# RoyAPTX4869/RaLD

Hardware: AMD Instinct MI355X
Metric: denoising steps/sec (whole node) (higher is better)
Workload: dtype bf16

## Files before the change

include/rald_hip.h:

```cpp
#ifndef RALD_HIP_H
#define RALD_HIP_H
#include <stdint.h>
#ifdef __cplusplus
extern "C" {
#endif

const char* rald_last_error(void);
int rald_version(void);
int rald_build_flags(void);
int64_t rald_debug_f16_saturation_count(int32_t reset);
int rald_debug_poison_lds(void* stream);

typedef struct rald_dit rald_dit;

typedef struct rald_dit_config {
    int32_t n_latents;
    int32_t channels;
    int32_t depth;
    int32_t n_heads;
    int32_t d_head;
    int32_t t_channels;
    int32_t context_dim;
    int32_t n_cond_tokens;
    int32_t with_radar_enc;
// ... 170 lines not shown
typedef struct rald_lidar rald_lidar;
int rald_lidar_create(const rald_lidar_config* cfg, rald_lidar** out);
void rald_lidar_destroy(rald_lidar* h);
int64_t rald_lidar_workspace_bytes(const rald_lidar_config* cfg, int32_t batch, int64_t total_points);
int rald_lidar_crop(const rald_lidar* h, const float* points, int32_t in_stride, const int64_t* offsets, int32_t batch, float* out,
                    int32_t* counts, void* workspace, int64_t workspace_bytes, void* stream);
int rald_lidar_voxelize(const rald_lidar* h, const float* points, const int64_t* offsets, const int32_t* counts, int32_t batch,
                        int32_t to_polar, float* polar_out, float* voxels, int32_t* coords, int32_t* num_points, int32_t* kept_keys,
                        int32_t* voxel_counts, void* workspace, int64_t workspace_bytes, void* stream);
int rald_lidar_queries(const rald_lidar* h, const float* points, const int64_t* offsets, int32_t batch, int32_t num_samples,
                       int32_t in_num, const int64_t* sample_idx, const double* u_in, const int64_t* voxel_idx, const double* u_out,
                       const int64_t* empty_rank, const int32_t* coords, const int32_t* kept_keys, const int32_t* voxel_counts,
                       float* lidar_points, float* query_points, float* query_labels, void* workspace, int64_t workspace_bytes,
                       void* stream);

int rald_op_gemm_nt(const void* A, int64_t lda, int64_t strideA, const void* B, int64_t ldb, int64_t strideB,
                    void* C, int64_t ldc, int64_t strideC, const float* bias, int32_t M, int32_t N, int32_t K,
                    int32_t batch, float alpha, int32_t epilogue, void* stream);
int rald_op_gemm_nt2(const void* A, int64_t lda, int64_t strideA, int64_t strideA2, const void* B, int64_t ldb, int64_t strideB, int64_t strideB2,
                     void* C, int64_t ldc, int64_t strideC, int64_t strideC2, const float* bias, int32_t M, int32_t N, int32_t K, int32_t batch,
                     int32_t batch2, float alpha, int32_t epilogue, void* stream);
int rald_op_gemm_nt_256(const void* A, int64_t lda, const void* B, int64_t ldb, void* C, int64_t ldc, const float* bias, int32_t M, int32_t N,
                        int32_t K, float alpha, int32_t alpha_ncols, int32_t epilogue, int32_t persistent, int32_t max_workgroups, void* stream);
int rald_op_gemm_tn(const void* A_bf16, int64_t lda, const void* B_bf16, int64_t ldb, float* C, int64_t ldc, float* colsum, int32_t M, int32_t N1,
                    int32_t N2, void* workspace, int64_t workspace_bytes, void* stream);
int rald_op_conv3d_wgrad(const void* dy_bf16, const void* x_bf16, float* dW, float* dbias, int32_t B, int32_t ID, int32_t IH, int32_t IW, int32_t Cin,
                         int32_t Cout, int32_t stride, int32_t pad, void* workspace, int64_t workspace_bytes, void* stream);
int64_t rald_op_gemm_tn_workspace_bytes(int32_t M, int32_t N1, int32_t N2);
int64_t rald_op_conv3d_wgrad_workspace_bytes(int32_t B, int32_t ID, int32_t IH, int32_t IW, int32_t Cin, int32_t Cout, int32_t stride, int32_t pad);
int rald_op_patches27(const float* cube, int32_t cube_ch, void* out_bf16, int32_t B, int32_t D, int32_t H, int32_t W, void* stream);
int rald_op_transpose(const void* in, int32_t in_is_bf16, int64_t ld_in, int64_t stride_in, int64_t stride_in2, void* out_bf16, int64_t ld_out,
                      int64_t stride_out, int64_t stride_out2, int32_t rows, int32_t cols, int32_t batch, int32_t batch2, void* stream);
int rald_op_ln_mod_bwd(const float* x, const float* dh, const float* scale, int64_t gstride, int32_t rows_per_group, float add_one, float eps,
                       int64_t rows, int32_t D, float* dx_accum, void* dx_bf16_out, float* dscale_accum, float* dshift_accum, void* stream);
int rald_op_geglu_fwd(const void* u_bf16, void* hid_bf16, int64_t M, int32_t inner, void* stream);
int rald_op_geglu_bwd(const void* u_bf16, const void* dhid_bf16, void* du_bf16, int64_t M, int32_t inner, void* stream);
int rald_op_colsum(const void* X, int32_t is_bf16, int64_t ld, int64_t M, int32_t N, float* out_accum, void* stream);
int rald_op_row_lse(const float* S, int64_t rows, int32_t cols, float scale, float* lse, void* stream);
int rald_op_rowdot_heads(const void* dO_bf16, const void* O_bf16, int64_t M, int32_t heads, int32_t nq, float* delta, void* stream);
int rald_op_attn_bwd_elem(const float* S, const float* dP, const float* lse, const float* delta, int64_t batch, int32_t R, int32_t Ccols,
                          int64_t vbatch_stride, int32_t vstride, float scale, int32_t by_col, void* P_bf16, void* dS_bf16, void* stream);
int rald_op_sgemm_acc(const float* A, int64_t lda, int32_t trans_a, const float* B, int64_t ldb, int32_t trans_b, float* C, int64_t ldc, int32_t M,
                      int32_t N, int32_t K, float alpha, void* stream);
int rald_op_silu_fwd(const float* x, float* y, int64_t n, void* stream);
int rald_op_silu_bwd(const float* x_pre, const float* dy, float* dx, int64_t n, void* stream);
int rald_op_posemb(const float* t, float* out, int32_t n, int32_t channels, void* stream);
// ... 129 lines not shown
```

rald_amd/_handles.py:

```python
from __future__ import annotations

import ctypes as C
import os
from typing import Dict, Iterable, Optional, Sequence, Tuple

import torch

from . import _lib
from ._lib import DitConfig, check, lib


def _stream() -> int:
    return torch.cuda.current_stream().cuda_stream


def _opt(t: Optional[torch.Tensor]) -> Optional[int]:
    return t.data_ptr() if t is not None else None


def _need_cuda(t: torch.Tensor, what: str) -> None:
    if not t.is_cuda:
        raise RuntimeError(f"rald_amd: {what} must live on the GPU (cuda tensor); this package has no CPU path")


# ... 316 lines not shown
    sB = B.stride(0) if B.dim() == 3 else 0
    nc = N // 2 if epilogue == 3 else N
    if epilogue == 2:
        out = C_inout
    else:
        shape = (batch, M, nc) if batched else (M, nc)
        out = torch.empty(shape, device=A.device, dtype=torch.float16 if epilogue == 5 else (torch.bfloat16 if epilogue in (0, 3, 4) else torch.float32))
    sC = out.stride(0) if out.dim() == 3 else 0
    check(lib().rald_op_gemm_nt(A.data_ptr(), A.stride(-2), sA, B.data_ptr(), B.stride(-2), sB, out.data_ptr(), out.stride(-2), sC, _opt(bias), M, N,
                                K, batch, alpha, epilogue, _stream()))
    return out


def op_gemm_nt_256(A: torch.Tensor, B: torch.Tensor, out: torch.Tensor, bias: Optional[torch.Tensor] = None, epilogue: int = 0, alpha: float = 1.0,
                   alpha_ncols: int = 1 << 30, persistent: int = 1, max_workgroups: int = 1 << 30) -> torch.Tensor:
    (M, K), N = A.shape, B.shape[0]
    assert A.dtype == B.dtype == out.dtype == torch.bfloat16 and A.stride(1) == B.stride(1) == out.stride(1) == 1
    assert out.shape == (M, N // 2 if epilogue == 3 else N) and B.shape[1] == K
    check(lib().rald_op_gemm_nt_256(A.data_ptr(), A.stride(0), B.data_ptr(), B.stride(0), out.data_ptr(), out.stride(0), _opt(bias), M, N, K,
                                    alpha, int(alpha_ncols), int(epilogue), int(persistent), int(max_workgroups), _stream()))
    return out


def op_gemm_tn(A: torch.Tensor, B: torch.Tensor, C_inout: torch.Tensor, colsum: Optional[torch.Tensor] = None, atomics: bool = True) -> torch.Tensor:
    M, N1 = A.shape
    N2 = B.shape[1]
    assert A.dtype == torch.bfloat16 and B.dtype == torch.bfloat16 and C_inout.dtype == torch.float32 and B.shape[0] == M
    assert A.stride(1) == 1 and B.stride(1) == 1 and C_inout.stride(1) == 1 and C_inout.shape == (N1, N2)
    ws, nbytes = None, 0
    if not atomics:
        nbytes = lib().rald_op_gemm_tn_workspace_bytes(M, N1, N2)
        ws = _scratch(nbytes, A.device)
    check(lib().rald_op_gemm_tn(A.data_ptr(), A.stride(0), B.data_ptr(), B.stride(0), C_inout.data_ptr(), C_inout.stride(0),
                                _opt(colsum), M, N1, N2, _opt(ws), nbytes, _stream()))
    return C_inout


def op_gemm_resid_ln(A: torch.Tensor, W: torch.Tensor, bias: torch.Tensor, x: torch.Tensor, g: torch.Tensor, b: torch.Tensor,
                     gstride: int = 0, rows_per_group: int = 1 << 30, add_one: float = 0.0, eps: float = 1e-5) -> torch.Tensor:
    M, K = A.shape
    h = torch.empty(M, 512, device=A.device, dtype=torch.bfloat16)
    check(lib().rald_op_gemm_resid_ln(A.data_ptr(), A.stride(0), W.data_ptr(), W.stride(0), bias.data_ptr(),
                                      x.data_ptr(), h.data_ptr(), g.data_ptr(), b.data_ptr(), gstride,
                                      rows_per_group, add_one, eps, M, K, _stream()))
    return h

# ... 368 lines not shown
```

rald_amd/csrc/api.hip:

```cpp
#include <cstdlib>
#include <cstring>

#include "ae.h"
#include "dit.h"
#include "lidar.h"
#include "radar_dsp.h"
#include "radar_points.h"

using namespace rald;

struct rald_dit { Dit impl; };
struct rald_ae { Ae impl; };

extern "C" {

const char* rald_last_error(void) { return rald::last_error(); }
int rald_version(void) { return 3; }
int rald_build_flags(void) { return 0; }

int64_t rald_debug_f16_saturation_count(int32_t reset) {
    unsigned a = 0, b = 0;
    if (hipDeviceSynchronize() != hipSuccess) return -1;
    if (f16_saturation_gemm(&a, reset != 0) || f16_saturation_attn(&b, reset != 0)) return -1;
    return (int64_t)a + (int64_t)b;
// ... 482 lines not shown
                    void* C, int64_t ldc, int64_t strideC, const float* bias, int32_t M, int32_t N, int32_t K,
                    int32_t batch, float alpha, int32_t epilogue, void* stream) {
    RALD_CHECK(A && B && C, "rald_op_gemm_nt: null pointer");
    GemmArgs g;
    g.A = (const bf16*)A; g.lda = lda; g.strideA = strideA; g.B = (const bf16*)B; g.ldb = ldb; g.strideB = strideB;
    g.C = C; g.ldc = ldc; g.strideC = strideC; g.bias = bias; g.M = M; g.N = N; g.K = K; g.batch = batch; g.alpha = alpha; g.alpha_ncols = 1 << 30; g.flags = 0;
    return gemm_nt(g, epilogue, (hipStream_t)stream);
}
int rald_op_gemm_nt2(const void* A, int64_t lda, int64_t strideA, int64_t strideA2, const void* B, int64_t ldb, int64_t strideB, int64_t strideB2,
                     void* C, int64_t ldc, int64_t strideC, int64_t strideC2, const float* bias, int32_t M, int32_t N, int32_t K, int32_t batch,
                     int32_t batch2, float alpha, int32_t epilogue, void* stream) {
    RALD_CHECK(A && B && C, "rald_op_gemm_nt2: null pointer");
    GemmArgs g = gemm_args((const bf16*)A, lda, (const bf16*)B, ldb, C, ldc, bias, M, N, K);
    g.strideA = strideA; g.strideB = strideB; g.strideC = strideC; g.batch = batch; g.alpha = alpha;
    g.batch2 = batch2; g.strideA2 = strideA2; g.strideB2 = strideB2; g.strideC2 = strideC2;
    return gemm_nt(g, epilogue, (hipStream_t)stream);
}
int rald_op_gemm_nt_256(const void* A, int64_t lda, const void* B, int64_t ldb, void* C, int64_t ldc, const float* bias, int32_t M, int32_t N,
                        int32_t K, float alpha, int32_t alpha_ncols, int32_t epilogue, int32_t persistent, int32_t max_workgroups, void* stream) {
    RALD_CHECK(A && B && C, "rald_op_gemm_nt_256: null pointer");
    GemmArgs g = gemm_args((const bf16*)A, lda, (const bf16*)B, ldb, C, ldc, bias, M, N, K);
    g.alpha = alpha; g.alpha_ncols = alpha_ncols;
    return gemm_nt_256_test(g, epilogue, persistent, max_workgroups, (hipStream_t)stream);
}
int rald_op_gemm_tn(const void* A_bf16, int64_t lda, const void* B_bf16, int64_t ldb, float* C, int64_t ldc, float* colsum, int32_t M, int32_t N1,
                    int32_t N2, void* workspace, int64_t workspace_bytes, void* stream) {
    return gemm_tn((const bf16*)A_bf16, lda, (const bf16*)B_bf16, ldb, C, ldc, colsum, M, N1, N2, (hipStream_t)stream, (float*)workspace, workspace_bytes / 4);
}
int rald_op_conv3d_wgrad(const void* dy_bf16, const void* x_bf16, float* dW, float* dbias, int32_t B, int32_t ID, int32_t IH, int32_t IW, int32_t Cin,
                         int32_t Cout, int32_t stride, int32_t pad, void* workspace, int64_t workspace_bytes, void* stream) {
    return conv3d_wgrad_tn((const bf16*)dy_bf16, (const bf16*)x_bf16, dW, dbias, B, ID, IH, IW, Cin, Cout, stride, pad, (hipStream_t)stream, (float*)workspace,
                           workspace_bytes / 4);
}
int64_t rald_op_gemm_tn_workspace_bytes(int32_t M, int32_t N1, int32_t N2) { return 4 * gemm_tn_workspace_floats(M, N1, N2); }
int64_t rald_op_conv3d_wgrad_workspace_bytes(int32_t B, int32_t ID, int32_t IH, int32_t IW, int32_t Cin, int32_t Cout, int32_t stride, int32_t pad) {
    return 4 * conv3d_wgrad_workspace_floats(B, ID, IH, IW, Cin, Cout, stride, pad);
}
int rald_op_patches27(const float* cube, int32_t cube_ch, void* out_bf16, int32_t B, int32_t D, int32_t H, int32_t W, void* stream) {
    return patches27(cube, cube_ch, (bf16*)out_bf16, B, D, H, W, (hipStream_t)stream);
}
int rald_op_transpose(const void* in, int32_t in_is_bf16, int64_t ld_in, int64_t stride_in, int64_t stride_in2, void* out_bf16, int64_t ld_out,
                      int64_t stride_out, int64_t stride_out2, int32_t rows, int32_t cols, int32_t batch, int32_t batch2, void* stream) {
    TransposeArgs a;
    a.in = in; a.ld_in = ld_in; a.stride_in = stride_in; a.stride_in2 = stride_in2; a.out = (bf16*)out_bf16; a.ld_out = ld_out;
    a.stride_out = stride_out; a.stride_out2 = stride_out2; a.rows = rows; a.cols = cols; a.batch = batch; a.batch2 = batch2;
    return transpose_rows(a, in_is_bf16, (hipStream_t)stream);
// ... 400 lines not shown
```

rald_amd/csrc/gemm.hip:

```cpp
#include <algorithm>
#include <cstdlib>
#include <type_traits>

#include "common.h"
#include "kernels.h"
#include "gemm_epilogue.h"
#include "gemm_tile.h"

namespace rald {

template <int MT, int NT, int EPI>
__device__ __forceinline__ void gemm_epilogue(f32x4 (&acc)[MT][NT], const GemmArgs& a, int mb, int nb, int64_t coff, int fr, int fq) {
    if constexpr (EPI == EPI_GEGLU) {
        bf16* C = reinterpret_cast<bf16*>(a.C) + coff;
#pragma unroll
        for (int i = 0; i < MT; ++i) {
            const int m = mb + i * 16 + fr;
            if (m >= a.M) continue;
#pragma unroll
            for (int p = 0; p < NT / 2; ++p) {
                const int nx = nb + 32 * p + 4 * fq;
                const int ng = nx + 16;
                float4 bx = *reinterpret_cast<const float4*>(a.bias + nx);
                float4 bg = *reinterpret_cast<const float4*>(a.bias + ng);
// ... 268 lines not shown
            else asm volatile("s_waitcnt vmcnt(0)" ::: "memory");
            asm volatile("" ::: "memory");
            __builtin_amdgcn_s_barrier();
            asm volatile("" ::: "memory");
            if (kt + NSTAGE - 1 < nk) stage(kt + NSTAGE - 1, (kt + NSTAGE - 1) % NSTAGE);
#pragma unroll
            for (int kk = 0; kk < 2; ++kk) {
                bf16x8 fa[MT], fb[NT];
                read_frags(kt % NSTAGE, kk, fa, fb);
                mfma_all(fa, fb);
            }
        }
    }
    if constexpr (NSTAGE != 2) {
        asm volatile("" ::: "memory");
        __builtin_amdgcn_s_barrier();
        asm volatile("" ::: "memory");
    }
    gemm_epilogue_lds<MT, NT, EPI>(acc, a, m0 + wm * (BM / WM), n0 + wn * (BN / WN), coff, lane, smem + wave * EPI_PATCH_BYTES,
                                   reinterpret_cast<float*>(smem + WAVES * EPI_PATCH_BYTES) + wave * NT * 16);
}

constexpr int PERSIST_LDS_BYTES = 160 * 1024;
template <int EPI>
__global__ __launch_bounds__(512) void gemm_nt_persist_kernel(GemmArgs a) {
    static_assert(EPI == EPI_BF16 || EPI == EPI_GEGLU, "the persistent engine is built for the two bf16-output epilogues");
    constexpr int BM = 256, BN = 256, BK = 64, WN = 2, MT = 4, NT = 8;
    constexpr int DW = 4;
    constexpr int CP = BM / 8 / DW;
    constexpr int STAGE_BYTES = (BM + BN) * BK * 2;
    constexpr int OC = (EPI == EPI_GEGLU) ? NT * 8 : NT * 16;
    constexpr int ROWB = OC * 2, STRIDE = ROWB + 16, LPR = ROWB / 16;
    constexpr int PR = (EPI == EPI_GEGLU) ? 16 : 8;
    constexpr int PATCH = PR * STRIDE;
    constexpr int RPI = 64 / LPR;
    constexpr int BIAS_OFF = 2 * STAGE_BYTES + 31 * 1024;
    static_assert(2 * STAGE_BYTES + 8 * PATCH <= BIAS_OFF && BIAS_OFF + BN * 4 <= PERSIST_LDS_BYTES && PR % RPI == 0, "LDS plan");
    extern __shared__ __attribute__((aligned(16))) unsigned char smem[];
    float* tbias = reinterpret_cast<float*>(smem + BIAS_OFF);

    const int tid = threadIdx.x;
    const int lane = tid & 63;
    const int wave = __builtin_amdgcn_readfirstlane(tid >> 6);
    const int wm = wave / WN, wn = wave % WN;
    const bool dma = wave < DW;
    const int ntm = a.M / BM, ntn = a.N / BN, nt = ntm * ntn;
    const int nk = a.K / BK;
    const int fr = lane & 15, fq = lane >> 4;

    const unsigned voA = (unsigned)((lane >> 3) * (int)a.lda + RALD_SWZ(lane >> 3, lane & 7) * 8) * 2u;
    const unsigned voB = (unsigned)((lane >> 3) * (int)a.ldb + RALD_SWZ(lane >> 3, lane & 7) * 8) * 2u;
    const unsigned lds0 = (unsigned)(uintptr_t)(lds_void*)smem;
    auto dma_piece = [&](const char* base, unsigned voff, unsigned lds) {
        asm volatile("s_nop 0\n\tglobal_load_lds_dwordx4 %0, %1" ::"v"(voff), "s"(base), "{m0}"(lds) : "memory");
    };
    auto stage = [&](int m0, int n0, int kt, int buf) {
        const char* pa = reinterpret_cast<const char*>(a.A) + ((int64_t)(m0 + 8 * wave) * a.lda + kt * BK) * 2;
        const char* pb = reinterpret_cast<const char*>(a.B) + ((int64_t)(n0 + 8 * wave) * a.ldb + kt * BK) * 2;
        const unsigned s = lds0 + buf * STAGE_BYTES + wave * 1024;
#pragma unroll
        for (int p = 0; p < CP; ++p) dma_piece(pa + (int64_t)p * (8 * DW * 2) * a.lda, voA, s + p * DW * 1024);
#pragma unroll
        for (int p = 0; p < CP; ++p) dma_piece(pb + (int64_t)p * (8 * DW * 2) * a.ldb, voB, s + BM * 128 + p * DW * 1024);
    };
    auto read_frags = [&](int buf, int kk, bf16x8 (&fa)[MT], bf16x8 (&fb)[NT]) {
        const bf16x8* sA = reinterpret_cast<const bf16x8*>(smem + buf * STAGE_BYTES);
        const bf16x8* sB = sA + BM * 8;
        const int chunk = kk * 4 + fq;
#pragma unroll
        for (int i = 0; i < MT; ++i) {
            const int r = wm * (MT * 16) + i * 16 + fr;
            fa[i] = sA[r * 8 + RALD_SWZ(r, chunk)];
        }
#pragma unroll
        for (int j = 0; j < NT; ++j) {
            const int r = wn * (NT * 16) + j * 16 + fr;
            fb[j] = sB[r * 8 + RALD_SWZ(r, chunk)];
        }
    };
    f32x4 acc[MT][NT];
    auto mfma_all = [&](const bf16x8 (&fa)[MT], const bf16x8 (&fb)[NT]) {
#pragma unroll
        for (int i = 0; i < MT; ++i)
#pragma unroll
            for (int j = 0; j < NT; ++j)
                acc[i][j] = __builtin_amdgcn_mfma_f32_16x16x32_bf16(fb[j], fa[i], acc[i][j], 0, 0, 0);
    };
    constexpr int W_ALL = 0x0070;
    constexpr int W_LGKM = 0xc07f;
    constexpr int W_ST1 = ((2 * CP) & 15) | (((2 * CP) >> 4) << 14) | 0x0070;
    auto hand_over = [&]() {
        if (dma) __builtin_amdgcn_s_waitcnt(W_ALL);
        else __builtin_amdgcn_s_waitcnt(W_LGKM);
        __builtin_amdgcn_s_barrier();
    };
    bf16x8 fa0[MT], fb0[NT], fa1[MT], fb1[NT];
    auto body = [&](int m0, int n0, int kt, bool with_dma) {
        const int cur = kt & 1;
        if (with_dma && dma) stage(m0, n0, kt + 1, cur ^ 1);
        __builtin_amdgcn_sched_barrier(0);
        read_frags(cur, 0, fa0, fb0);
        mfma_all(fa1, fb1);
#pragma unroll
        for (int g = 0; g < 12; ++g) {
            __builtin_amdgcn_sched_group_barrier(0x008, 2, 0);
            __builtin_amdgcn_sched_group_barrier(0x100, 1, 0);
        }
        __builtin_amdgcn_sched_group_barrier(0x008, 8, 0);
        __builtin_amdgcn_sched_barrier(0);
        read_frags(cur, 1, fa1, fb1);
        mfma_all(fa0, fb0);
#pragma unroll
        for (int g = 0; g < 12; ++g) {
            __builtin_amdgcn_sched_group_barrier(0x008, 2, 0);
            __builtin_amdgcn_sched_group_barrier(0x100, 1, 0);
        }
        __builtin_amdgcn_sched_group_barrier(0x008, 8, 0);
        __builtin_amdgcn_sched_barrier(0);
        hand_over();
    };

    if (!a.bias && tid < BN / 4) *reinterpret_cast<float4*>(tbias + 4 * tid) = make_float4(0.f, 0.f, 0.f, 0.f);
    int t = blockIdx.x;
    int tm, tn;
    xcd_strip_tile_at(t, ntn, ntm, tm, tn);
    int m0 = tm * BM, n0 = tn * BN;
    if (dma) {
        stage(m0, n0, 0, 0);
        if (nk > 1) stage(m0, n0, 1, 1);
    }
    for (;;) {
#pragma unroll
        for (int i = 0; i < MT; ++i)
#pragma unroll
            for (int j = 0; j < NT; ++j) acc[i][j] = f32x4{0.f, 0.f, 0.f, 0.f};
        if (dma) {
            if (nk > 1) __builtin_amdgcn_s_waitcnt(W_ST1);
            else __builtin_amdgcn_s_waitcnt(W_ALL);
        } else __builtin_amdgcn_s_waitcnt(W_LGKM);
        __builtin_amdgcn_s_barrier();
        if (wave == 0 && a.bias) dma_piece(reinterpret_cast<const char*>(a.bias + n0), 16u * lane, lds0 + BIAS_OFF);
        read_frags(0, 0, fa0, fb0);
        read_frags(0, 1, fa1, fb1);
        mfma_all(fa0, fb0);
        hand_over();
        for (int kt = 1; kt + 1 < nk; ++kt) body(m0, n0, kt, true);
        if (nk > 1) body(m0, n0, nk - 1, false);
        const int tnext = t + gridDim.x;
        int m0n = 0, n0n = 0;
        if (tnext < nt) {
            xcd_strip_tile_at(tnext, ntn, ntm, tm, tn);
            m0n = tm * BM;
            n0n = tn * BN;
            if (dma) {
                stage(m0n, n0n, 0, 0);
                if (nk > 1) stage(m0n, n0n, 1, 1);
            }
        }
        mfma_all(fa1, fb1);

        {
            int lane_e = lane;
            asm volatile("" : "+v"(lane_e));
            const int fr = lane_e & 15, fq = lane_e >> 4;
            unsigned char* patch = smem + 2 * STAGE_BYTES + wave * PATCH;
            const int mb = m0 + wm * (MT * 16), nb = n0 + wn * (NT * 16);
            const int oc0 = (EPI == EPI_GEGLU) ? nb / 2 : nb;
            const float* wbias = tbias + wn * (NT * 16);
            bf16* C = reinterpret_cast<bf16*>(a.C);
#pragma unroll
            for (int i = 0; i < MT; ++i) {
#pragma unroll
                for (int h = 0; h < 16 / PR; ++h) {
                    asm volatile("" ::: "memory");
                    if (PR == 16 || (fr >> 3) == h) {
                        const int pr = fr & (PR - 1);
                        if constexpr (EPI == EPI_GEGLU) {
#pragma unroll
                            for (int p = 0; p < NT / 2; ++p) {
                                const float4 bx = *reinterpret_cast<const float4*>(wbias + 32 * p + 4 * fq);
                                const float4 bg = *reinterpret_cast<const float4*>(wbias + 32 * p + 4 * fq + 16);
                                const f32x4 x = acc[i][2 * p], g = acc[i][2 * p + 1];
                                const f32x2 g01 = gelu_poly2(f32x2{g[0] + bg.x, g[1] + bg.y});
                                const f32x2 g23 = gelu_poly2(f32x2{g[2] + bg.z, g[3] + bg.w});
                                const f32x2 o01 = f32x2{x[0] + bx.x, x[1] + bx.y} * g01;
                                const f32x2 o23 = f32x2{x[2] + bx.z, x[3] + bx.w} * g23;
                                *reinterpret_cast<bf16x4*>(patch + pr * STRIDE + (16 * p + 4 * fq) * 2) = pack4(o01[0], o01[1], o23[0], o23[1]);
                            }
                        } else {
#pragma unroll
                            for (int j = 0; j < NT; ++j) {
                                const int n = nb + j * 16 + 4 * fq;
                                const float4 b = *reinterpret_cast<const float4*>(wbias + 16 * j + 4 * fq);
                                const f32x4 v = acc[i][j];
                                const float al = n < a.alpha_ncols ? a.alpha : 1.0f;
                                const float o0 = al * v[0] + b.x, o1 = al * v[1] + b.y, o2 = al * v[2] + b.z, o3 = al * v[3] + b.w;
                                *reinterpret_cast<bf16x4*>(patch + pr * STRIDE + (16 * j + 4 * fq) * 2) = pack4(o0, o1, o2, o3);
                            }
                        }
                    }
                    asm volatile("" ::: "memory");
                    __builtin_amdgcn_s_waitcnt(W_LGKM);
                    __builtin_amdgcn_s_barrier();
                    asm volatile("" ::: "memory");
                    if (!dma) {
                        const int r = lane_e / LPR, pc = lane_e % LPR;
                        uint4 v[2][PR / RPI];
#pragma unroll
                        for (int w2 = 0; w2 < 2; ++w2)
#pragma unroll
                            for (int q = 0; q < PR / RPI; ++q)
                                v[w2][q] = *reinterpret_cast<const uint4*>(patch - w2 * DW * PATCH + (q * RPI + r) * STRIDE + pc * 16);
#pragma unroll
                        for (int w2 = 0; w2 < 2; ++w2)
#pragma unroll
                            for (int q = 0; q < PR / RPI; ++q) {
                                const int m = mb - w2 * (BM / 2) + i * 16 + h * PR + q * RPI + r;
                                bf16* Cp = C + (int64_t)m * a.ldc + oc0 + pc * 8;
                                typedef unsigned int u32x4 __attribute__((ext_vector_type(4)));
                                const u32x4 vv = u32x4{v[w2][q].x, v[w2][q].y, v[w2][q].z, v[w2][q].w};
                                asm volatile("global_store_dwordx4 %0, %1, off sc0 sc1 nt\n\ts_nop 1" ::"v"(Cp), "v"(vv) : "memory");
                            }
                    }
                    asm volatile("" ::: "memory");
                    __builtin_amdgcn_s_waitcnt(W_LGKM);
                    __builtin_amdgcn_s_barrier();
                    asm volatile("" ::: "memory");
                }
            }
        }
        if (tnext >= nt) break;
        t = tnext;
        m0 = m0n;
        n0 = n0n;
    }
}

template <int BM, int BN>
static int launch_tile(const GemmArgs& a, int epi, hipStream_t st) {
    dim3 grid(cdiv(a.N, BN), cdiv(a.M, BM), a.batch * a.batch2);
    switch (epi) {
        case EPI_BF16:  hipLaunchKernelGGL((gemm_nt_kernel<BM, BN, EPI_BF16>), grid, dim3(256), 0, st, a); break;
        case EPI_F32:   hipLaunchKernelGGL((gemm_nt_kernel<BM, BN, EPI_F32>), grid, dim3(256), 0, st, a); break;
        case EPI_RESID: hipLaunchKernelGGL((gemm_nt_kernel<BM, BN, EPI_RESID>), grid, dim3(256), 0, st, a); break;
        case EPI_GEGLU: hipLaunchKernelGGL((gemm_nt_kernel<BM, BN, EPI_GEGLU>), grid, dim3(256), 0, st, a); break;
        default: set_error("gemm: bad epilogue"); return 1;
    }
    RALD_HIP(hipGetLastError());
    return 0;
}

template <int BM, int BN, int WM, int WN, int NSTAGE, int EPI>
static int launch_glds_epi(const GemmArgs& a, hipStream_t st) {
    constexpr int WAVES = WM * WN;
    constexpr int smem = NSTAGE * (BM + BN) * 64 * 2;
    static_assert(smem >= epi_lds_bytes<BN / (16 * WN)>(WAVES), "epilogue patches and bias slots must fit in the staging buffers");
    static bool raised = false;
// ... 8 lines not shown
        case EPI_GEGLU: return launch_glds_epi<BM, BN, WM, WN, NSTAGE, EPI_GEGLU>(a, st);
        case EPI_F16S:
            if constexpr ((BM == 64 && BN == 64) || (BM == 128 && BN == 128 && NSTAGE == 2)) return launch_glds_epi<BM, BN, WM, WN, NSTAGE, EPI_F16S>(a, st);
            else { set_error("gemm: the fp16-slab epilogue is built for the 64x64 ring and the 128x128 LDS-DMA engines"); return 1; }
        case EPI_SOFTMAX64:
            if constexpr ((BN / WN) % 64 == 0 && BM >= 128) return launch_glds_epi<BM, BN, WM, WN, NSTAGE, EPI_SOFTMAX64>(a, st);
            else { set_error("gemm: the softmax epilogue needs waves of 64-column groups"); return 1; }
        default: set_error("gemm: bad epilogue"); return 1;
    }
}

static int cu_count(int& cus) {
    static int cached[64] = {};
    int dev = 0;
    RALD_HIP(hipGetDevice(&dev));
    RALD_CHECK(dev >= 0 && dev < 64, "gemm: device index out of range");
    if (cached[dev] == 0) RALD_HIP(hipDeviceGetAttribute(&cached[dev], hipDeviceAttributeMultiprocessorCount, dev));
    cus = cached[dev];
    return 0;
}
static int launch_persist(const GemmArgs& a, int epi, int max_workgroups, hipStream_t st) {
    int cus = 0;
    if (int rc = cu_count(cus)) return rc;
    const int64_t tiles = (int64_t)(a.M / 256) * (a.N / 256);
    const int grid = (int)std::min<int64_t>(tiles, std::min(cus, max_workgroups));
    RALD_CHECK(grid >= 1, "gemm: the persistent engine needs at least one workgroup");
    static bool raised_bf16 = false, raised_geglu = false;
    switch (epi) {
        case EPI_BF16:  return launch_dyn_lds(gemm_nt_persist_kernel<EPI_BF16>, raised_bf16, dim3(grid), 512, PERSIST_LDS_BYTES, st, a);
        case EPI_GEGLU: return launch_dyn_lds(gemm_nt_persist_kernel<EPI_GEGLU>, raised_geglu, dim3(grid), 512, PERSIST_LDS_BYTES, st, a);
        default: set_error("gemm: the persistent engine has the bf16 and GEGLU epilogues"); return 1;
    }
}

int f16_saturation_gemm(unsigned* count, bool reset) {
    RALD_HIP(hipMemcpyFromSymbol(count, HIP_SYMBOL(g_f16_sat_gemm), sizeof(unsigned)));
    if (reset) { const unsigned z = 0; RALD_HIP(hipMemcpyToSymbol(HIP_SYMBOL(g_f16_sat_gemm), &z, sizeof(unsigned))); }
    return 0;
}

int gemm_nt(const GemmArgs& a0, int epi, hipStream_t st) {
    GemmArgs a = a0;
    a.flags |= GEMM_NT_STORE;
    RALD_CHECK(a.M > 0 && a.N > 0 && a.K > 0 && a.batch > 0 && a.batch2 > 0, "gemm: empty problem");
    const int64_t nbatch = (int64_t)a.batch * a.batch2;
    RALD_CHECK(nbatch <= 65535, "gemm: batch * batch2 exceeds the grid z limit");
    RALD_CHECK(a.K % 64 == 0, "gemm: K must be a multiple of 64 (pad with zeros)");
    RALD_CHECK(a.N % 4 == 0, "gemm: N must be a multiple of 4");
    RALD_CHECK(a.lda % 8 == 0 && a.ldb % 8 == 0, "gemm: lda/ldb must be multiples of 8 elements (16-byte rows)");
    RALD_CHECK(a.lda >= a.K && a.ldb >= a.K, "gemm: leading dimension smaller than K");
    RALD_CHECK(((uintptr_t)a.A % 16 == 0) && ((uintptr_t)a.B % 16 == 0) && ((uintptr_t)a.C % 16 == 0), "gemm: pointers must be 16-byte aligned");
    RALD_CHECK(a.ldc % 4 == 0, "gemm: ldc must be a multiple of 4");
    if (epi == EPI_GEGLU) {
        RALD_CHECK(a.N % 128 == 0 && a.bias != nullptr, "gemm: GEGLU needs N % 128 == 0 and a packed bias");
        RALD_CHECK(a.ldc >= a.N / 2, "gemm: GEGLU ldc < N/2");
    } else {
        RALD_CHECK(a.ldc >= a.N, "gemm: ldc < N");
    }
    if (epi == EPI_F16S) {
        RALD_CHECK(!a.out8 && a.N % 8 == 0, "gemm: the fp16-slab epilogue needs N % 8 == 0");
        const int64_t w128 = (int64_t)cdiv(a.M, 128) * cdiv(a.N, 128) * nbatch, w64 = (int64_t)cdiv(a.M, 64) * cdiv(a.N, 64) * nbatch;
        RALD_CHECK(w128 >= 192 || w64 <= 256, "gemm: fp16 slabs are not built for the register-staged engine (ask gemm_f16s_ok first)");
        if (w128 >= 192) return launch_glds<128, 128, 2, 2, 2>(a, epi, st);
        return launch_glds<64, 64, 2, 2, 8>(a, epi, st);
    }
    if (epi == EPI_SOFTMAX64) {
        RALD_CHECK(a.M % 128 == 0 && a.N % 128 == 0 && !a.bias && !a.out8 && a.alpha_ncols >= a.N, "gemm: the softmax epilogue needs M, N % 128 == 0 and no bias");
        if (a.M % 256 == 0 && a.N % 256 == 0 && (int64_t)(a.M / 256) * (a.N / 256) * nbatch >= 256) return launch_glds<256, 256, 4, 2, 2>(a, epi, st);
        return launch_glds<128, 128, 2, 2, 2>(a, epi, st);
    }
    if (a.out8) {
        RALD_CHECK(epi == EPI_GEGLU && a.outs && a.batch * a.batch2 == 1 && a.M % 256 == 0 && a.N % 256 == 0 && (a.N / 2) % 32 == 0 &&
                   (int64_t)(a.M / 256) * (a.N / 256) >= 256, "gemm: the MXFP8 output form needs the GEGLU epilogue on full 256x256 tiles");
        return launch_glds<256, 256, 4, 2, 2>(a, epi, st);
    }
    const int64_t wg128 = (int64_t)cdiv(a.M, 128) * cdiv(a.N, 128) * nbatch;
    if (wg128 < 192) {
        const int64_t wg64 = (int64_t)cdiv(a.M, 64) * cdiv(a.N, 64) * nbatch;
        if (wg64 > 256) return launch_tile<64, 64>(a, epi, st);
        return launch_glds<64, 64, 2, 2, 8>(a, epi, st);
    }
    const int64_t wg256 = (int64_t)(a.M / 256) * (a.N / 256) * nbatch;
    if (a.M % 256 == 0 && a.N % 256 == 0 && wg256 >= 256) {
        if (nbatch == 1 && (epi == EPI_BF16 || epi == EPI_GEGLU)) {
            int cus = 0;
            if (int rc = cu_count(cus)) return rc;
            if (wg256 >= 2 * (int64_t)cus) return launch_persist(a, epi, 1 << 30, st);
        }
        return launch_glds<256, 256, 4, 2, 2>(a, epi, st);
    }
    if (epi != EPI_GEGLU && wg128 <= 320 && a.M % 64 == 0) return launch_glds<64, 128, 2, 2, 3>(a, epi, st);
    return launch_glds<128, 128, 2, 2, 2>(a, epi, st);
}

int gemm_nt_256_test(const GemmArgs& a0, int epi, int persistent, int max_workgroups, hipStream_t st) {
    GemmArgs a = a0;
    a.flags |= GEMM_NT_STORE;
    RALD_CHECK(epi == EPI_BF16 || epi == EPI_GEGLU, "gemm_nt_256_test: EPI_BF16 or EPI_GEGLU");
    RALD_CHECK(a.M > 0 && a.N > 0 && a.K > 0 && a.M % 256 == 0 && a.N % 256 == 0 && a.K % 64 == 0, "gemm_nt_256_test: M, N % 256 == 0 and K % 64 == 0");
    RALD_CHECK(a.batch == 1 && a.batch2 == 1 && !a.out8, "gemm_nt_256_test: one problem, bf16 output");
    RALD_CHECK(a.lda % 8 == 0 && a.ldb % 8 == 0 && a.lda >= a.K && a.ldb >= a.K, "gemm_nt_256_test: lda/ldb must be multiples of 8 and at least K");
    RALD_CHECK(((uintptr_t)a.A % 16 == 0) && ((uintptr_t)a.B % 16 == 0) && ((uintptr_t)a.C % 16 == 0) && ((uintptr_t)a.bias % 16 == 0),
               "gemm_nt_256_test: pointers must be 16-byte aligned");
    RALD_CHECK(a.ldc % 8 == 0 && a.ldc >= (epi == EPI_GEGLU ? a.N / 2 : a.N), "gemm_nt_256_test: ldc");
    RALD_CHECK(epi != EPI_GEGLU || a.bias, "gemm_nt_256_test: GEGLU needs a packed bias");
    RALD_CHECK(max_workgroups >= 1, "gemm_nt_256_test: max_workgroups must be at least 1");
    if (persistent) return launch_persist(a, epi, max_workgroups, st);
    return launch_glds<256, 256, 4, 2, 2>(a, epi, st);
}

}
```

rald_amd/csrc/kernels.h:

```cpp
#pragma once
#include <cstdlib>
#include <vector>

#include "common.h"

namespace rald {

enum { GEMM_NT_STORE = 64 };
enum { EPI_BF16 = 0, EPI_F32 = 1, EPI_RESID = 2, EPI_GEGLU = 3,
       EPI_SOFTMAX64 = 4,
       EPI_F16S = 5 };
struct GemmArgs {
    const bf16* A; int64_t lda; int64_t strideA;
    const bf16* B; int64_t ldb; int64_t strideB;
    void* C;       int64_t ldc; int64_t strideC;
    const float* bias;
    int M, N, K, batch;
    float alpha;
    int alpha_ncols;
    int flags;
    int batch2 = 1;
    int64_t strideA2 = 0, strideB2 = 0, strideC2 = 0;
    unsigned char *out8 = nullptr, *outs = nullptr;
};
#ifdef __HIPCC__
__device__ __forceinline__ void gemm_batch_offsets(const GemmArgs& a, int bz, int64_t& oa, int64_t& ob, int64_t& oc) {
    const int b1 = bz / a.batch2, b2 = bz - b1 * a.batch2;
    oa = (int64_t)b1 * a.strideA + (int64_t)b2 * a.strideA2;
    ob = (int64_t)b1 * a.strideB + (int64_t)b2 * a.strideB2;
    oc = (int64_t)b1 * a.strideC + (int64_t)b2 * a.strideC2;
}
#endif
int gemm_nt(const GemmArgs& a, int epi, hipStream_t st);
int gemm_nt_256_test(const GemmArgs& a, int epi, int persistent, int max_workgroups, hipStream_t st);
int f16_saturation_gemm(unsigned* count, bool reset);
int f16_saturation_attn(unsigned* count, bool reset);
inline bool gemm_f16s_ok(int M, int N, int batch) {
    const int64_t w128 = (int64_t)((M + 127) / 128) * ((N + 127) / 128) * batch, w64 = (int64_t)((M + 63) / 64) * ((N + 63) / 64) * batch;
    return w128 >= 192 || w64 <= 256;
}
inline GemmArgs gemm_args(const bf16* A, int64_t lda, const bf16* B, int64_t ldb, void* C, int64_t ldc,
                          const float* bias, int M, int N, int K) {
    GemmArgs g;
    g.A = A; g.lda = lda; g.strideA = 0; g.B = B; g.ldb = ldb; g.strideB = 0;
    g.C = C; g.ldc = ldc; g.strideC = 0; g.bias = bias; g.M = M; g.N = N; g.K = K; g.batch = 1; g.alpha = 1.f; g.alpha_ncols = 1 << 30; g.flags = 0;
    return g;
}

struct GemmLnArgs {
    const bf16* A; int64_t lda;
    const bf16* W; int64_t ldw;
    const float* bias;
    float* x;
    bf16* h;
    unsigned char* h8 = nullptr;
    unsigned char* hs = nullptr;
    int nt_io = 1;
// ... 280 lines not shown
```

Before: 5933.

## Route batched softmax GEMM through persistent engine with double-buffered epilogue patches

Extends the persistent 256x256 GEMM kernel to handle batched problems with the fused softmax epilogue, using a batch-aware tile scheduler. gemm_nt routes softmax GEMMs there when there are at least two tiles per CU. The epilogue store also moves to alternating LDS patch slots, which removes the second barrier per store step. The aim is to overlap the next tile's loads with the epilogue and cut launch and tail cost, at the risk of LDS hazards between slots and a different tile order for batched work.

```diff
diff --git a/include/rald_hip.h b/include/rald_hip.h
--- a/include/rald_hip.h
+++ b/include/rald_hip.h
@@ -216,6 +216,9 @@
                      int32_t batch2, float alpha, int32_t epilogue, void* stream);
 int rald_op_gemm_nt_256(const void* A, int64_t lda, const void* B, int64_t ldb, void* C, int64_t ldc, const float* bias, int32_t M, int32_t N,
                         int32_t K, float alpha, int32_t alpha_ncols, int32_t epilogue, int32_t persistent, int32_t max_workgroups, void* stream);
+int rald_op_gemm_nt_256_batched(const void* A, int64_t lda, int64_t strideA, const void* B, int64_t ldb, int64_t strideB, void* C, int64_t ldc,
+                                int64_t strideC, const float* bias, int32_t M, int32_t N, int32_t K, int32_t batch, int32_t batch2, float alpha,
+                                int32_t alpha_ncols, int32_t epilogue, int32_t persistent, int32_t max_workgroups, void* stream);
 int rald_op_gemm_tn(const void* A_bf16, int64_t lda, const void* B_bf16, int64_t ldb, float* C, int64_t ldc, float* colsum, int32_t M, int32_t N1,
                     int32_t N2, void* workspace, int64_t workspace_bytes, void* stream);
 int rald_op_conv3d_wgrad(const void* dy_bf16, const void* x_bf16, float* dW, float* dbias, int32_t B, int32_t ID, int32_t IH, int32_t IW, int32_t Cin,
diff --git a/rald_amd/_handles.py b/rald_amd/_handles.py
--- a/rald_amd/_handles.py
+++ b/rald_amd/_handles.py
@@ -362,6 +362,19 @@
     return out
 
 
+def op_gemm_nt_256_batched(A: torch.Tensor, B: torch.Tensor, out: torch.Tensor, bias: Optional[torch.Tensor] = None, epilogue: int = 0,
+                           alpha: float = 1.0, alpha_ncols: int = 1 << 30, persistent: int = 1, max_workgroups: int = 1 << 30) -> torch.Tensor:
+    batch, M, nc = out.shape
+    K, N = A.shape[-1], B.shape[-2]
+    assert A.dtype == B.dtype == out.dtype == torch.bfloat16 and A.stride(-1) == B.stride(-1) == out.stride(-1) == 1
+    assert A.shape[-2] == M and B.shape[-1] == K and nc == (N // 2 if epilogue == 3 else N)
+    assert all(t.dim() == 2 or t.shape[0] == batch for t in (A, B))
+    check(lib().rald_op_gemm_nt_256_batched(A.data_ptr(), A.stride(-2), A.stride(0) if A.dim() == 3 else 0, B.data_ptr(), B.stride(-2),
+                                            B.stride(0) if B.dim() == 3 else 0, out.data_ptr(), out.stride(-2), out.stride(0), _opt(bias), M, N, K,
+                                            batch, 1, alpha, int(alpha_ncols), int(epilogue), int(persistent), int(max_workgroups), _stream()))
+    return out
+
+
 def op_gemm_tn(A: torch.Tensor, B: torch.Tensor, C_inout: torch.Tensor, colsum: Optional[torch.Tensor] = None, atomics: bool = True) -> torch.Tensor:
     M, N1 = A.shape
     N2 = B.shape[1]
diff --git a/rald_amd/csrc/api.hip b/rald_amd/csrc/api.hip
--- a/rald_amd/csrc/api.hip
+++ b/rald_amd/csrc/api.hip
@@ -528,6 +528,15 @@
     GemmArgs g = gemm_args((const bf16*)A, lda, (const bf16*)B, ldb, C, ldc, bias, M, N, K);
     g.alpha = alpha; g.alpha_ncols = alpha_ncols;
     return gemm_nt_256_test(g, epilogue, persistent, max_workgroups, (hipStream_t)stream);
+}
+int rald_op_gemm_nt_256_batched(const void* A, int64_t lda, int64_t strideA, const void* B, int64_t ldb, int64_t strideB, void* C, int64_t ldc,
+                                int64_t strideC, const float* bias, int32_t M, int32_t N, int32_t K, int32_t batch, int32_t batch2, float alpha,
+                                int32_t alpha_ncols, int32_t epilogue, int32_t persistent, int32_t max_workgroups, void* stream) {
+    RALD_CHECK(A && B && C, "rald_op_gemm_nt_256_batched: null pointer");
+    GemmArgs g = gemm_args((const bf16*)A, lda, (const bf16*)B, ldb, C, ldc, bias, M, N, K);
+    g.strideA = strideA; g.strideB = strideB; g.strideC = strideC; g.batch = batch; g.batch2 = batch2;
+    g.alpha = alpha; g.alpha_ncols = alpha_ncols;
+    return gemm_nt_256_batched_test(g, epilogue, persistent, max_workgroups, (hipStream_t)stream);
 }
 int rald_op_gemm_tn(const void* A_bf16, int64_t lda, const void* B_bf16, int64_t ldb, float* C, int64_t ldc, float* colsum, int32_t M, int32_t N1,
                     int32_t N2, void* workspace, int64_t workspace_bytes, void* stream) {
diff --git a/rald_amd/csrc/gemm.hip b/rald_amd/csrc/gemm.hip
--- a/rald_amd/csrc/gemm.hip
+++ b/rald_amd/csrc/gemm.hip
@@ -314,9 +314,23 @@
 }
 
 constexpr int PERSIST_LDS_BYTES = 160 * 1024;
+__device__ __forceinline__ void batched_tile_at(int g, int ntn, int ntm, int nbatch, int& bz, int& tm, int& tn) {
+    const int nt = ntn * ntm;
+    if (nt < 8 && (nbatch & 7) == 0) {
+        const int slot = g >> 3;
+        bz = (slot / nt) * 8 + (g & 7);
+        const int tl = slot % nt;
+        tm = tl / ntn;
+        tn = tl % ntn;
+    } else {
+        bz = g / nt;
+        xcd_strip_tile_at(g - bz * nt, ntn, ntm, tm, tn);
+    }
+}
 template <int EPI>
 __global__ __launch_bounds__(512) void gemm_nt_persist_kernel(GemmArgs a) {
-    static_assert(EPI == EPI_BF16 || EPI == EPI_GEGLU, "the persistent engine is built for the two bf16-output epilogues");
+    static_assert(EPI == EPI_BF16 || EPI == EPI_GEGLU || EPI == EPI_SOFTMAX64, "the persistent engine is built for the three bf16-output epilogues");
+    constexpr bool BATCHED = EPI == EPI_SOFTMAX64, BIAS = EPI != EPI_SOFTMAX64;
     constexpr int BM = 256, BN = 256, BK = 64, WN = 2, MT = 4, NT = 8;
     constexpr int DW = 4;
     constexpr int CP = BM / 8 / DW;
@@ -325,9 +339,11 @@
     constexpr int ROWB = OC * 2, STRIDE = ROWB + 16, LPR = ROWB / 16;
     constexpr int PR = (EPI == EPI_GEGLU) ? 16 : 8;
     constexpr int PATCH = PR * STRIDE;
+    constexpr int NSLOT = 12;
     constexpr int RPI = 64 / LPR;
     constexpr int BIAS_OFF = 2 * STAGE_BYTES + 31 * 1024;
-    static_assert(2 * STAGE_BYTES + 8 * PATCH <= BIAS_OFF && BIAS_OFF + BN * 4 <= PERSIST_LDS_BYTES && PR % RPI == 0, "LDS plan");
+    static_assert(2 * STAGE_BYTES + NSLOT * PATCH <= BIAS_OFF && BIAS_OFF + BN * 4 <= PERSIST_LDS_BYTES && PR % RPI == 0 && (MT * 16 / PR) % 2 == 0,
+                  "LDS plan; an even number of steps per tile keeps the slot parity across tiles");
     extern __shared__ __attribute__((aligned(16))) unsigned char smem[];
     float* tbias = reinterpret_cast<float*>(smem + BIAS_OFF);
 
@@ -336,7 +352,7 @@
     const int wave = __builtin_amdgcn_readfirstlane(tid >> 6);
     const int wm = wave / WN, wn = wave % WN;
     const bool dma = wave < DW;
-    const int ntm = a.M / BM, ntn = a.N / BN, nt = ntm * ntn;
+    const int ntm = a.M / BM, ntn = a.N / BN, nt = ntm * ntn * (BATCHED ? a.batch : 1);
     const int nk = a.K / BK;
     const int fr = lane & 15, fq = lane >> 4;
 
@@ -346,9 +362,16 @@
     auto dma_piece = [&](const char* base, unsigned voff, unsigned lds) {
         asm volatile("s_nop 0\n\tglobal_load_lds_dwordx4 %0, %1" ::"v"(voff), "s"(base), "{m0}"(lds) : "memory");
     };
-    auto stage = [&](int m0, int n0, int kt, int buf) {
-        const char* pa = reinterpret_cast<const char*>(a.A) + ((int64_t)(m0 + 8 * wave) * a.lda + kt * BK) * 2;
-        const char* pb = reinterpret_cast<const char*>(a.B) + ((int64_t)(n0 + 8 * wave) * a.ldb + kt * BK) * 2;
+    struct Tile { int64_t oa, ob, oc; int m0, n0; };
+    auto tile_at = [&](int t) {
+        int bz = 0, tm, tn;
+        if constexpr (BATCHED) batched_tile_at(t, ntn, ntm, a.batch, bz, tm, tn);
+        else xcd_strip_tile_at(t, ntn, ntm, tm, tn);
+        return Tile{bz * a.strideA, bz * a.strideB, bz * a.strideC, tm * BM, tn * BN};
+    };
+    auto stage = [&](const Tile& T, int kt, int buf) {
+        const char* pa = reinterpret_cast<const char*>(a.A) + (T.oa + (int64_t)(T.m0 + 8 * wave) * a.lda + kt * BK) * 2;
+        const char* pb = reinterpret_cast<const char*>(a.B) + (T.ob + (int64_t)(T.n0 + 8 * wave) * a.ldb + kt * BK) * 2;
         const unsigned s = lds0 + buf * STAGE_BYTES + wave * 1024;
 #pragma unroll
         for (int p = 0; p < CP; ++p) dma_piece(pa + (int64_t)p * (8 * DW * 2) * a.lda, voA, s + p * DW * 1024);
@@ -387,9 +410,9 @@
         __builtin_amdgcn_s_barrier();
     };
     bf16x8 fa0[MT], fb0[NT], fa1[MT], fb1[NT];
-    auto body = [&](int m0, int n0, int kt, bool with_dma) {
+    auto body = [&](const Tile& T, int kt, bool with_dma) {
         const int cur = kt & 1;
-        if (with_dma && dma) stage(m0, n0, kt + 1, cur ^ 1);
+        if (with_dma && dma) stage(T, kt + 1, cur ^ 1);
         __builtin_amdgcn_sched_barrier(0);
         read_frags(cur, 0, fa0, fb0);
         mfma_all(fa1, fb1);
@@ -412,14 +435,13 @@
         hand_over();
     };
 
-    if (!a.bias && tid < BN / 4) *reinterpret_cast<float4*>(tbias + 4 * tid) = make_float4(0.f, 0.f, 0.f, 0.f);
+    if constexpr (BIAS)
+        if (!a.bias && tid < BN / 4) *reinterpret_cast<float4*>(tbias + 4 * tid) = make_float4(0.f, 0.f, 0.f, 0.f);
     int t = blockIdx.x;
-    int tm, tn;
-    xcd_strip_tile_at(t, ntn, ntm, tm, tn);
-    int m0 = tm * BM, n0 = tn * BN;
+    Tile T = tile_at(t);
     if (dma) {
-        stage(m0, n0, 0, 0);
-        if (nk > 1) stage(m0, n0, 1, 1);
+        stage(T, 0, 0);
+        if (nk > 1) stage(T, 1, 1);
     }
     for (;;) {
 #pragma unroll
@@ -431,22 +453,21 @@
             else __builtin_amdgcn_s_waitcnt(W_ALL);
         } else __builtin_amdgcn_s_waitcnt(W_LGKM);
         __builtin_amdgcn_s_barrier();
-        if (wave == 0 && a.bias) dma_piece(reinterpret_cast<const char*>(a.bias + n0), 16u * lane, lds0 + BIAS_OFF);
+        if constexpr (BIAS)
+            if (wave == 0 && a.bias) dma_piece(reinterpret_cast<const char*>(a.bias + T.n0), 16u * lane, lds0 + BIAS_OFF);
         read_frags(0, 0, fa0, fb0);
         read_frags(0, 1, fa1, fb1);
         mfma_all(fa0, fb0);
         hand_over();
-        for (int kt = 1; kt + 1 < nk; ++kt) body(m0, n0, kt, true);
-        if (nk > 1) body(m0, n0, nk - 1, false);
+        for (int kt = 1; kt + 1 < nk; ++kt) body(T, kt, true);
+        if (nk > 1) body(T, nk - 1, false);
         const int tnext = t + gridDim.x;
-        int m0n = 0, n0n = 0;
+        Tile Tn = T;
         if (tnext < nt) {
-            xcd_strip_tile_at(tnext, ntn, ntm, tm, tn);
-            m0n = tm * BM;
-            n0n = tn * BN;
+            Tn = tile_at(tnext);
             if (dma) {
-                stage(m0n, n0n, 0, 0);
-                if (nk > 1) stage(m0n, n0n, 1, 1);
+                stage(Tn, 0, 0);
+                if (nk > 1) stage(Tn, 1, 1);
             }
         }
         mfma_all(fa1, fb1);
@@ -455,15 +476,40 @@
             int lane_e = lane;
             asm volatile("" : "+v"(lane_e));
             const int fr = lane_e & 15, fq = lane_e >> 4;
-            unsigned char* patch = smem + 2 * STAGE_BYTES + wave * PATCH;
-            const int mb = m0 + wm * (MT * 16), nb = n0 + wn * (NT * 16);
+            unsigned char* slot0 = smem + 2 * STAGE_BYTES + wave * PATCH;
+            unsigned char* slot1 = slot0 + (dma ? 8 * PATCH : 0);
+            const int mb = T.m0 + wm * (MT * 16), nb = T.n0 + wn * (NT * 16);
             const int oc0 = (EPI == EPI_GEGLU) ? nb / 2 : nb;
             const float* wbias = tbias + wn * (NT * 16);
-            bf16* C = reinterpret_cast<bf16*>(a.C);
+            bf16* C = reinterpret_cast<bf16*>(a.C) + T.oc;
 #pragma unroll
             for (int i = 0; i < MT; ++i) {
+                bf16x4 sm[EPI == EPI_SOFTMAX64 ? NT : 1];
+                if constexpr (EPI == EPI_SOFTMAX64) {
+#pragma unroll
+                    for (int g = 0; g < NT / 4; ++g) {
+                        float e[16];
+                        float mx = -3.0e38f;
+#pragma unroll
+                        for (int q = 0; q < 4; ++q)
+#pragma unroll
+                            for (int c = 0; c < 4; ++c) { e[4 * q + c] = a.alpha * acc[i][4 * g + q][c]; mx = fmaxf(mx, e[4 * q + c]); }
+                        mx = fmaxf(mx, __shfl_xor(mx, 16, 64));
+                        mx = fmaxf(mx, __shfl_xor(mx, 32, 64));
+                        float su = 0.f;
+#pragma unroll
+                        for (int q = 0; q < 16; ++q) { e[q] = __builtin_amdgcn_exp2f(e[q] - mx); su += e[q]; }
+                        su += __shfl_xor(su, 16, 64);
+                        su += __shfl_xor(su, 32, 64);
+                        const float inv = 1.0f / su;
+#pragma unroll
+                        for (int q = 0; q < 4; ++q) sm[4 * g + q] = pack4(e[4 * q] * inv, e[4 * q + 1] * inv, e[4 * q + 2] * inv, e[4 * q + 3] * inv);
+                    }
+                }
 #pragma unroll
                 for (int h = 0; h < 16 / PR; ++h) {
+                    const int odd = (i * (16 / PR) + h) & 1;
+                    unsigned char* patch = odd ? slot1 : slot0;
                     asm volatile("" ::: "memory");
                     if (PR == 16 || (fr >> 3) == h) {
                         const int pr = fr & (PR - 1);
@@ -479,6 +525,9 @@
                                 const f32x2 o23 = f32x2{x[2] + bx.z, x[3] + bx.w} * g23;
                                 *reinterpret_cast<bf16x4*>(patch + pr * STRIDE + (16 * p + 4 * fq) * 2) = pack4(o01[0], o01[1], o23[0], o23[1]);
                             }
+                        } else if constexpr (EPI == EPI_SOFTMAX64) {
+#pragma unroll
+                            for (int j = 0; j < NT; ++j) *reinterpret_cast<bf16x4*>(patch + pr * STRIDE + (16 * j + 4 * fq) * 2) = sm[j];
                         } else {
 #pragma unroll
                             for (int j = 0; j < NT; ++j) {
@@ -493,16 +542,20 @@
                     }
                     asm volatile("" ::: "memory");
                     __builtin_amdgcn_s_waitcnt(W_LGKM);
+                    asm volatile("" ::: "memory");
+                    const int r = lane_e / LPR, pc = lane_e % LPR;
+                    uint4 v[2][PR / RPI];
+                    if (!dma) {
+#pragma unroll
+                        for (int q = 0; q < PR / RPI; ++q) v[0][q] = *reinterpret_cast<const uint4*>(slot0 + (q * RPI + r) * STRIDE + pc * 16);
+                    }
+                    asm volatile("" ::: "memory");
                     __builtin_amdgcn_s_barrier();
                     asm volatile("" ::: "memory");
                     if (!dma) {
-                        const int r = lane_e / LPR, pc = lane_e % LPR;
-                        uint4 v[2][PR / RPI];
-#pragma unroll
-                        for (int w2 = 0; w2 < 2; ++w2)
-#pragma unroll
-                            for (int q = 0; q < PR / RPI; ++q)
-                                v[w2][q] = *reinterpret_cast<const uint4*>(patch - w2 * DW * PATCH + (q * RPI + r) * STRIDE + pc * 16);
+                        const unsigned char* partner = slot0 - DW * PATCH + (odd ? 8 * PATCH : 0);
+#pragma unroll
+                        for (int q = 0; q < PR / RPI; ++q) v[1][q] = *reinterpret_cast<const uint4*>(partner + (q * RPI + r) * STRIDE + pc * 16);
 #pragma unroll
                         for (int w2 = 0; w2 < 2; ++w2)
 #pragma unroll
@@ -515,16 +568,12 @@
                             }
                     }
                     asm volatile("" ::: "memory");
-                    __builtin_amdgcn_s_waitcnt(W_LGKM);
-                    __builtin_amdgcn_s_barrier();
-                    asm volatile("" ::: "memory");
                 }
             }
         }
         if (tnext >= nt) break;
         t = tnext;
-        m0 = m0n;
-        n0 = n0n;
+        T = Tn;
     }
 }
 
@@ -579,14 +628,16 @@
 static int launch_persist(const GemmArgs& a, int epi, int max_workgroups, hipStream_t st) {
     int cus = 0;
     if (int rc = cu_count(cus)) return rc;
-    const int64_t tiles = (int64_t)(a.M / 256) * (a.N / 256);
+    const int64_t tiles = (int64_t)(a.M / 256) * (a.N / 256) * a.batch;
+    RALD_CHECK(tiles < (1ll << 30), "gemm: too many tiles for the persistent engine's tile index");
     const int grid = (int)std::min<int64_t>(tiles, std::min(cus, max_workgroups));
     RALD_CHECK(grid >= 1, "gemm: the persistent engine needs at least one workgroup");
-    static bool raised_bf16 = false, raised_geglu = false;
+    static bool raised_bf16 = false, raised_geglu = false, raised_softmax = false;
     switch (epi) {
+        case EPI_SOFTMAX64: return launch_dyn_lds(gemm_nt_persist_kernel<EPI_SOFTMAX64>, raised_softmax, dim3(grid), 512, PERSIST_LDS_BYTES, st, a);
         case EPI_BF16:  return launch_dyn_lds(gemm_nt_persist_kernel<EPI_BF16>, raised_bf16, dim3(grid), 512, PERSIST_LDS_BYTES, st, a);
         case EPI_GEGLU: return launch_dyn_lds(gemm_nt_persist_kernel<EPI_GEGLU>, raised_geglu, dim3(grid), 512, PERSIST_LDS_BYTES, st, a);
-        default: set_error("gemm: the persistent engine has the bf16 and GEGLU epilogues"); return 1;
+        default: set_error("gemm: the persistent engine has the bf16, GEGLU and softmax epilogues"); return 1;
     }
 }
 
@@ -623,7 +674,15 @@
     }
     if (epi == EPI_SOFTMAX64) {
         RALD_CHECK(a.M % 128 == 0 && a.N % 128 == 0 && !a.bias && !a.out8 && a.alpha_ncols >= a.N, "gemm: the softmax epilogue needs M, N % 128 == 0 and no bias");
-        if (a.M % 256 == 0 && a.N % 256 == 0 && (int64_t)(a.M / 256) * (a.N / 256) * nbatch >= 256) return launch_glds<256, 256, 4, 2, 2>(a, epi, st);
+        if (a.M % 256 == 0 && a.N % 256 == 0) {
+            const int64_t wg256 = (int64_t)(a.M / 256) * (a.N / 256) * nbatch;
+            if (a.batch2 == 1) {
+                int cus = 0;
+                if (int rc = cu_count(cus)) return rc;
+                if (wg256 >= 2 * (int64_t)cus) return launch_persist(a, epi, 1 << 30, st);
+            }
+            if (wg256 >= 256) return launch_glds<256, 256, 4, 2, 2>(a, epi, st);
+        }
         return launch_glds<128, 128, 2, 2, 2>(a, epi, st);
     }
     if (a.out8) {
@@ -666,4 +725,28 @@
     return launch_glds<256, 256, 4, 2, 2>(a, epi, st);
 }
 
-}
+int gemm_nt_256_batched_test(const GemmArgs& a0, int epi, int persistent, int max_workgroups, hipStream_t st) {
+    GemmArgs a = a0;
+    a.flags |= GEMM_NT_STORE;
+    RALD_CHECK(epi == EPI_BF16 || epi == EPI_GEGLU || epi == EPI_SOFTMAX64, "gemm_nt_256_batched_test: EPI_BF16, EPI_GEGLU or EPI_SOFTMAX64");
+    RALD_CHECK(a.M > 0 && a.N > 0 && a.K > 0 && a.M % 256 == 0 && a.N % 256 == 0 && a.K % 64 == 0,
+               "gemm_nt_256_batched_test: M, N % 256 == 0 and K % 64 == 0 (full tiles only)");
+    RALD_CHECK(a.batch >= 1 && a.batch <= 65535 && !a.out8, "gemm_nt_256_batched_test: 1 <= batch <= 65535, bf16 output");
+    RALD_CHECK(a.batch2 == 1, "gemm_nt_256_batched_test: batch2 must be 1 (the engine has no inner batch)");
+    RALD_CHECK(a.lda % 8 == 0 && a.ldb % 8 == 0 && a.lda >= a.K && a.ldb >= a.K, "gemm_nt_256_batched_test: lda/ldb must be multiples of 8 and at least K");
+    RALD_CHECK(((uintptr_t)a.A % 16 == 0) && ((uintptr_t)a.B % 16 == 0) && ((uintptr_t)a.C % 16 == 0) && ((uintptr_t)a.bias % 16 == 0),
+               "gemm_nt_256_batched_test: pointers must be 16-byte aligned");
+    const int ncols = epi == EPI_GEGLU ? a.N / 2 : a.N;
+    RALD_CHECK(a.ldc % 8 == 0 && a.ldc >= ncols, "gemm_nt_256_batched_test: ldc");
+    RALD_CHECK(a.strideA >= 0 && a.strideB >= 0 && a.strideA % 8 == 0 && a.strideB % 8 == 0 && a.strideC % 8 == 0,
+               "gemm_nt_256_batched_test: strides must be non-negative multiples of 8 elements");
+    RALD_CHECK(a.batch == 1 || a.strideC >= (int64_t)(a.M - 1) * a.ldc + ncols, "gemm_nt_256_batched_test: strideC lets the outputs of two entries overlap");
+    RALD_CHECK(epi != EPI_GEGLU || a.bias, "gemm_nt_256_batched_test: GEGLU needs a packed bias");
+    RALD_CHECK(epi != EPI_SOFTMAX64 || (!a.bias && a.alpha_ncols >= a.N), "gemm_nt_256_batched_test: the softmax epilogue takes no bias and one alpha");
+    RALD_CHECK(max_workgroups >= 1, "gemm_nt_256_batched_test: max_workgroups must be at least 1");
+    RALD_CHECK(!persistent || a.batch == 1 || epi == EPI_SOFTMAX64, "gemm_nt_256_batched_test: the persistent engine is batched for EPI_SOFTMAX64 only");
+    if (persistent) return launch_persist(a, epi, max_workgroups, st);
+    return launch_glds<256, 256, 4, 2, 2>(a, epi, st);
+}
+
+}
diff --git a/rald_amd/csrc/kernels.h b/rald_amd/csrc/kernels.h
--- a/rald_amd/csrc/kernels.h
+++ b/rald_amd/csrc/kernels.h
@@ -33,6 +33,7 @@
 #endif
 int gemm_nt(const GemmArgs& a, int epi, hipStream_t st);
 int gemm_nt_256_test(const GemmArgs& a, int epi, int persistent, int max_workgroups, hipStream_t st);
+int gemm_nt_256_batched_test(const GemmArgs& a, int epi, int persistent, int max_workgroups, hipStream_t st);
 int f16_saturation_gemm(unsigned* count, bool reset);
 int f16_saturation_attn(unsigned* count, bool reset);
 inline bool gemm_f16s_ok(int M, int N, int batch) {
```

Result: faster. 5999, median of 6 (+1.1%).
